# IvoteSligte/raytracing_engine

Measured on AMD Instinct MI355X. Metric: Mrays/s, higher is better.
Workload: dtype f32; 1 GPU; tri1m_1080p_4spp: 1000000 random triangles (edge +-0.08) + 1 emissive quad, single-level compressed BVH8 (249155 nodes, depth 9, one-triangle leaves), 1920x1080, 4 spp, 1 bounce + NEE, path B wavefront path tracer (camera rays: packet kernel); width=1920, height=1080, spp=4, bounces=1, tile=64, persistent_workgroups_per_cu=context default (7 for a whole frame), parallelism=single GPU, frames_in_flight=3

## Files before the change

raytracing_engine_amd/csrc/bvh_build.cpp:

```cpp
#include "bvh_build.h"

#include <algorithm>
#include <atomic>
#include <cmath>
#include <cstring>
#include <exception>
#include <limits>
#include <system_error>
#include <thread>

#include "bvh_node.h"
#include "host_parallel.h"

#ifdef RT_BVH_TIMING
#include <chrono>
#include <cstdio>
#define RT_BVH_T(x) const auto x = std::chrono::steady_clock::now()
#define RT_BVH_REPORT(what, a, b) std::fprintf(stderr, "bvh: %-18s %8.1f ms\n", what, std::chrono::duration<double, std::milli>((b) - (a)).count())
#else
#define RT_BVH_T(x) (void)0
#define RT_BVH_REPORT(what, a, b) (void)0
#endif

namespace rt {
namespace {

constexpr int kBins = 16;

struct Builder {
    const std::vector<Box>& tri_boxes;
    const std::vector<float>& centroid;
    std::vector<uint32_t>& order;
    std::vector<float>& nodes;
    float pad;
    uint32_t max_depth;
    uint32_t kLeafMax = 4;
    std::atomic<int>* spare_threads = nullptr;
    int n_threads = 1;

    struct Sub {
        int32_t ref;
        uint32_t depth_reached;
        double sah;
    };

    Box range_box(uint32_t first, uint32_t count) const {
        Box b = Box::empty();
        for (uint32_t i = 0; i < count; i++) b.grow(tri_boxes[order[first + i]]);
        return b;
    }

    void write_node(uint32_t me, const Box& b0, int32_t r0, const Box& b1, int32_t r1) {
        float* n = &nodes[(size_t)me * 16];
        const Box* side[2] = {&b0, &b1};
        for (int s = 0; s < 2; s++)
            for (int a = 0; a < 3; a++) {
                n[6 * s + a] = side[s]->lo[a] - pad;
                n[6 * s + 3 + a] = side[s]->hi[a] + pad;
            }
        std::memcpy(&n[12], &r0, 4);
        std::memcpy(&n[13], &r1, 4);
        n[14] = n[15] = 0.0f;
    }

    static int32_t leaf_ref(uint32_t first, uint32_t count) { return ~(int32_t)((first << 2) | (count - 1u)); }

    uint32_t min_depth(uint32_t count) const {
        uint32_t d = 0;
        uint64_t cap = kLeafMax;
        while (cap < count) {
            cap <<= 1;
            d++;
        }
        return d;
    }

    Sub build(uint32_t first, uint32_t count, uint32_t depth, uint32_t me) {
        if (count <= kLeafMax) return Sub{leaf_ref(first, count), 0u, 0.0};

        const int par = count >= kParallelBinMin ? n_threads : 1;
        const size_t n_chunks = (size_t)std::max(par, 1);
        const uint32_t chunk = (uint32_t)((count + n_chunks - 1) / n_chunks);
        float clo[3], chi[3];
        {
            float one_lo[3], one_hi[3];
            std::vector<float> many_lo, many_hi;
            if (n_chunks > 1) {
                many_lo.resize(3 * n_chunks);
                many_hi.resize(3 * n_chunks);
            }
            float* plo = n_chunks > 1 ? many_lo.data() : one_lo;
            float* phi = n_chunks > 1 ? many_hi.data() : one_hi;
            for (size_t i = 0; i < 3 * n_chunks; i++) {
                plo[i] = std::numeric_limits<float>::infinity();
                phi[i] = -std::numeric_limits<float>::infinity();
            }
            parallel_for(n_chunks, par, 1, [&](size_t c) {
                float lo[3] = {plo[3 * c], plo[3 * c + 1], plo[3 * c + 2]}, hi[3] = {phi[3 * c], phi[3 * c + 1], phi[3 * c + 2]};
                const uint32_t i1 = std::min<uint32_t>(count, (uint32_t)(c + 1) * chunk);
                for (uint32_t i = (uint32_t)c * chunk; i < i1; i++) {
                    const float* ce = &centroid[3 * (size_t)order[first + i]];
                    for (int a = 0; a < 3; a++) {
                        lo[a] = std::min(lo[a], ce[a]);
                        hi[a] = std::max(hi[a], ce[a]);
                    }
                }
                for (int a = 0; a < 3; a++) {
                    plo[3 * c + a] = lo[a];
                    phi[3 * c + a] = hi[a];
                }
            });
            for (int a = 0; a < 3; a++) {
                clo[a] = plo[a];
                chi[a] = phi[a];
                for (size_t c = 1; c < n_chunks; c++) {
                    clo[a] = std::min(clo[a], plo[3 * c + a]);
                    chi[a] = std::max(chi[a], phi[3 * c + a]);
                }
            }
        }

        uint32_t mid = 0;
        const bool must_balance = depth + 1 + min_depth((count + 1) / 2) >= max_depth;
        if (!must_balance) {
            float best_cost = std::numeric_limits<float>::infinity();
            int best_axis = -1, best_bin = -1;
            struct Bins {
                Box bb[3][kBins];
                uint32_t bc[3][kBins];
            };
            Bins one_part;
            std::vector<Bins> many_part;
            if (n_chunks > 1) many_part.resize(n_chunks);
            Bins* part = n_chunks > 1 ? many_part.data() : &one_part;
            float kk[3];
            for (int a = 0; a < 3; a++) kk[a] = chi[a] - clo[a] > 0.0f ? (float)kBins / (chi[a] - clo[a]) : 0.0f;
            parallel_for(n_chunks, par, 1, [&](size_t c) {
                Bins& P = part[c];
                for (int a = 0; a < 3; a++)
                    for (int b = 0; b < kBins; b++) {
                        P.bb[a][b] = Box::empty();
                        P.bc[a][b] = 0;
                    }
                const uint32_t i1 = std::min<uint32_t>(count, (uint32_t)(c + 1) * chunk);
                for (uint32_t i = (uint32_t)c * chunk; i < i1; i++) {
                    const uint32_t t = order[first + i];
                    for (int a = 0; a < 3; a++) {
                        if (!(kk[a] > 0.0f)) continue;
                        int bin = (int)((centroid[3 * (size_t)t + a] - clo[a]) * kk[a]);
                        bin = std::min(std::max(bin, 0), kBins - 1);
                        P.bb[a][bin].grow(tri_boxes[t]);
                        P.bc[a][bin]++;
                    }
                }
            });
            for (int a = 0; a < 3; a++) {
                if (!(kk[a] > 0.0f)) continue;
                Box bb[kBins];
                uint32_t bc[kBins];
                for (int b = 0; b < kBins; b++) {
                    bb[b] = part[0].bb[a][b];
                    bc[b] = part[0].bc[a][b];
                    for (size_t c = 1; c < n_chunks; c++) {
                        bb[b].grow(part[c].bb[a][b]);
                        bc[b] += part[c].bc[a][b];
                    }
                }
                float right_area[kBins];
                uint32_t right_cnt[kBins];
                Box acc = Box::empty();
                uint32_t cnt = 0;
                for (int b = kBins - 1; b > 0; b--) {
                    acc.grow(bb[b]);
                    cnt += bc[b];
                    right_area[b] = cnt ? acc.half_area() : 0.0f;
                    right_cnt[b] = cnt;
                }
                acc = Box::empty();
                cnt = 0;
                for (int b = 0; b < kBins - 1; b++) {
                    acc.grow(bb[b]);
                    cnt += bc[b];
                    if (cnt == 0 || right_cnt[b + 1] == 0) continue;
                    const float cost = acc.half_area() * (float)cnt + right_area[b + 1] * (float)right_cnt[b + 1];
                    if (cost < best_cost) {
                        best_cost = cost;
                        best_axis = a;
                        best_bin = b;
                    }
                }
            }
            if (best_axis >= 0) {
                const float k = (float)kBins / (chi[best_axis] - clo[best_axis]);
                const float lo = clo[best_axis];
                auto it = std::partition(order.begin() + first, order.begin() + first + count, [&](uint32_t t) {
                    int bin = (int)((centroid[3 * (size_t)t + best_axis] - lo) * k);
                    bin = std::min(std::max(bin, 0), kBins - 1);
                    return bin <= best_bin;
                });
                mid = (uint32_t)(it - (order.begin() + first));
                if (depth + 1 + min_depth(std::max(mid, count - mid)) >= max_depth) mid = 0;
            }
        }
        if (mid == 0 || mid == count) {
            int axis = 0;
            if (chi[1] - clo[1] > chi[axis] - clo[axis]) axis = 1;
            if (chi[2] - clo[2] > chi[axis] - clo[axis]) axis = 2;
            mid = count / 2;
            std::nth_element(order.begin() + first, order.begin() + first + mid, order.begin() + first + count,
                             [&](uint32_t x, uint32_t y) {
                                 const float cx = centroid[3 * (size_t)x + axis], cy = centroid[3 * (size_t)y + axis];
                                 return cx < cy || (cx == cy && x < y);
                             });
        }

        Box b0 = range_box(first, mid), b1 = range_box(first + mid, count - mid);
        Sub s0, s1;
        bool forked = false;
        if (spare_threads && count >= kForkMin) {
            if (spare_threads->fetch_sub(1) > 0) {
                std::exception_ptr left_err;
                std::thread left;
                try {
                    left = std::thread([&]() noexcept {
                        try {
                            s0 = build(first, mid, depth + 1, me + 1u);
                        } catch (...) {
                            left_err = std::current_exception();
                        }
                    });
                    forked = true;
                } catch (const std::system_error&) {
                }
                if (forked) {
                    {
                        struct Join {
                            std::thread& t;
                            ~Join() {
                                if (t.joinable()) t.join();
                            }
                        } join{left};
                        try {
                            s1 = build(first + mid, count - mid, depth + 1, me + mid);
                        } catch (...) {
                            spare_threads->fetch_add(1);
                            throw;
                        }
                    }
                    spare_threads->fetch_add(1);
                    if (left_err) std::rethrow_exception(left_err);
                } else {
                    spare_threads->fetch_add(1);
                }
            } else {
                spare_threads->fetch_add(1);
            }
        }
        if (!forked) {
            s0 = build(first, mid, depth + 1, me + 1u);
            s1 = build(first + mid, count - mid, depth + 1, me + mid);
        }
        write_node(me, b0, s0.ref, b1, s1.ref);
        return Sub{(int32_t)me, std::max(depth, std::max(s0.depth_reached, s1.depth_reached)),
                   ((double)b0.half_area() + (double)b1.half_area()) + (s0.sah + s1.sah)};
    }
    static constexpr uint32_t kForkMin = 1u << 14;
    static constexpr uint32_t kParallelBinMin = 1u << 17;
};

}

namespace {

struct Child {
    Box box;
    int32_t ref;
};

struct Cw8Builder {
    const std::vector<float>& n2;
    const std::vector<uint32_t>& order2;
    std::vector<uint32_t>& nodes;
    std::vector<uint32_t>& order8;
    uint32_t depth = 0;

    static constexpr float kCostNode = 1.0f;
    float kCostPrim = 0.8f;
    struct Dp {
        float cost[8];
        uint8_t split[9];
        uint8_t prev;
        uint8_t is_leaf;
        uint32_t first, prims;
        Box box;
    };
    std::vector<Dp> dp;
    int max_threads = 0;
    int thread_count() const { return max_threads > 0 ? std::min(max_threads, host_threads()) : host_threads(); }

    Box child_box(int32_t node2, int side) const {
        Box b;
        std::memcpy(b.lo, &n2[(size_t)node2 * 16 + 6 * side], 12);
        std::memcpy(b.hi, &n2[(size_t)node2 * 16 + 6 * side + 3], 12);
        return b;
    }
    int32_t child_ref(int32_t node2, int side) const {
        int32_t r;
        std::memcpy(&r, &n2[(size_t)node2 * 16 + 12 + side], 4);
        return r;
    }

    void solve() {
        const size_t n_nodes = n2.size() / 16;
        dp.resize(n_nodes);
        const int threads = thread_count();
        struct Range {
            size_t lo, hi;
        };
        std::vector<Range> subtrees;
        std::vector<size_t> top;
        const size_t grain = std::max<size_t>(n_nodes / (size_t)(8 * threads), 4096);
        std::vector<Range> todo{Range{0, n_nodes}};
        while (!todo.empty()) {
            const Range r = todo.back();
            todo.pop_back();
            if (r.hi - r.lo <= grain || threads == 1) {
                subtrees.push_back(r);
                continue;
            }
            top.push_back(r.lo);
            const int32_t r0 = child_ref((int32_t)r.lo, 0), r1 = child_ref((int32_t)r.lo, 1);
            if (r0 >= 0 && r1 >= 0) {
                todo.push_back(Range{(size_t)r0, (size_t)r1});
                todo.push_back(Range{(size_t)r1, r.hi});
            } else if (r0 >= 0) {
                todo.push_back(Range{(size_t)r0, r.hi});
            } else if (r1 >= 0) {
                todo.push_back(Range{(size_t)r1, r.hi});
            }
        }
        parallel_for(subtrees.size(), threads, 1, [&](size_t i) {
            for (size_t jj = subtrees[i].hi; jj-- > subtrees[i].lo;) solve_node(jj);
        });
        std::sort(top.begin(), top.end());
        for (size_t i = top.size(); i-- > 0;) solve_node(top[i]);
    }

    void solve_node(size_t jj) {
        {
            const int32_t j = (int32_t)jj;
            Dp& d = dp[jj];
            Box cb[2];
            float carea[2];
            int32_t cr[2];
            uint32_t cprims[2], cfirst[2];
            for (int s = 0; s < 2; s++) {
                cb[s] = child_box(j, s);
                cr[s] = child_ref(j, s);
                carea[s] = cb[s].half_area();
                if (cr[s] < 0) {
                    const uint32_t ref = ~(uint32_t)cr[s];
                    cfirst[s] = ref >> 2;
                    cprims[s] = (ref & 3u) + 1u;
                } else {
                    cfirst[s] = dp[cr[s]].first;
                    cprims[s] = dp[cr[s]].prims;
                }
            }
            auto C = [&](int s, int i) -> float {
                if (cr[s] < 0) return carea[s] * (float)cprims[s] * kCostPrim;
                return dp[cr[s]].cost[i > 7 ? 7 : i];
            };
            d.box = cb[0];
            d.box.grow(cb[1]);
            const bool same = cr[0] < 0 && cr[0] == cr[1];
            d.first = std::min(cfirst[0], cfirst[1]);
            d.prims = same ? cprims[0] : cprims[0] + cprims[1];
            float D[9];
            D[1] = std::numeric_limits<float>::infinity();
            for (int i = 2; i <= 8; i++) {
                float best = std::numeric_limits<float>::infinity();
                int bk = 1;
                for (int k = 1; k < i; k++) {
                    const float c = C(0, k) + C(1, i - k);
                    if (c < best) {
                        best = c;
                        bk = k;
                    }
                }
                D[i] = best;
                d.split[i] = (uint8_t)bk;
            }
            const float area = d.box.half_area();
            const float c_leaf = d.prims <= 1 ? area * (float)d.prims * kCostPrim : std::numeric_limits<float>::infinity();
            const float c_int = D[8] + area * kCostNode;
            d.is_leaf = c_leaf <= c_int;
            d.cost[1] = d.is_leaf ? c_leaf : c_int;
            d.prev = 0;
            for (int i = 2; i <= 7; i++) {
                if (d.cost[i - 1] <= D[i]) {
                    d.cost[i] = d.cost[i - 1];
                    d.prev |= (uint8_t)(1u << i);
                } else {
                    d.cost[i] = D[i];
                }
            }
            d.cost[0] = 0.0f;
        }
    }

    void expand(int32_t ref, const Box& box, int budget, Child* out, int& k) const {
        if (ref < 0) {
            out[k].box = box;
            out[k++].ref = ref;
            return;
        }
        const Dp& d = dp[ref];
        if (budget > 7) budget = 7;
        while (budget > 1 && ((d.prev >> budget) & 1)) budget--;
        if (budget == 1) {
            out[k].box = d.box;
            out[k++].ref = d.is_leaf ? ~(int32_t)((d.first << 2) | (d.prims - 1u)) : ref;
            return;
        }
        distribute(ref, budget, out, k);
    }
    void distribute(int32_t node2, int budget, Child* out, int& k) const {
        const int kl = dp[node2].split[budget];
        const Box b0 = child_box(node2, 0), b1 = child_box(node2, 1);
        const int32_t r0 = child_ref(node2, 0), r1 = child_ref(node2, 1);
        if (r0 < 0 && r0 == r1) {
            expand(r0, b0, 1, out, k);
            return;
        }
        expand(r0, b0, kl, out, k);
        expand(r1, b1, budget - kl, out, k);
    }

    struct Pending {
        int32_t node2;
        uint32_t index, level;
    };
    struct Work {
        Pending pd;
        Child ch[8];
        int k;
        int child_in[8];
        Box box;
        uint32_t n_inner, n_tris;
        uint32_t child_base, tri_base;
    };

    void plan(const Pending& pd, Work& w) const {
        w.pd = pd;
        Child* ch = w.ch;
        int k = 0;
        if (dp[pd.node2].is_leaf && pd.level == 0) {
            const Dp& d = dp[pd.node2];
            ch[0].box = d.box;
            ch[0].ref = ~(int32_t)((d.first << 2) | (d.prims - 1u));
            k = 1;
        } else {
            distribute(pd.node2, 8, ch, k);
        }
        w.k = k;
        Box cb[8];
        w.box = Box::empty();
        for (int i = 0; i < k; i++) {
            cb[i] = ch[i].box;
            w.box.grow(cb[i]);
        }
        assign_slots(cb, k, w.box, w.child_in);
        w.n_inner = w.n_tris = 0;
        for (int s = 0; s < 8; s++) {
            const int i = w.child_in[s];
            if (i < 0) continue;
            if (ch[i].ref >= 0) w.n_inner++;
            else w.n_tris += (~(uint32_t)ch[i].ref & 3u) + 1u;
        }
    }

    void write(const Work& wk, Pending* next_level, uint32_t next_level_base) {
        const Child* ch = wk.ch;
        Box cb[8];
        uint32_t imask = 0, leafmask = 0, rank = 0, off = 0;
        for (int s = 0; s < 8; s++) {
            const int i = wk.child_in[s];
            if (i < 0) continue;
            cb[s] = ch[i].box;
            if (ch[i].ref >= 0) {
                imask |= 1u << s;
                next_level[wk.child_base + rank - next_level_base] = Pending{ch[i].ref, wk.child_base + rank, wk.pd.level + 1};
                rank++;
            } else {
                const uint32_t ref = ~(uint32_t)ch[i].ref, first = ref >> 2;
                leafmask |= 1u << s;
                order8[(size_t)wk.tri_base + off] = order2[first];
                off += 1;
            }
        }
        uint32_t* w = node_at(nodes.data(), wk.pd.index);
        quantise(wk.box, cb, imask | leafmask, w);
        node_set_topology(w, imask, wk.child_base, wk.tri_base, leafmask);
    }

    void build() {
        RT_BVH_T(t0);
        solve();
        RT_BVH_T(t1);
        RT_BVH_REPORT("  collapse: DP", t0, t1);
        const int threads = thread_count();
        nodes.clear();
        order8.clear();
        std::vector<Pending> level{Pending{0, 0, 0}}, next;
        std::vector<Work> work;
        uint32_t node_count = 1, tri_count = 0;
        depth = 0;
        while (!level.empty()) {
            depth = level[0].level + 1;
            work.resize(level.size());
            parallel_for(level.size(), threads, 256, [&](size_t i) { plan(level[i], work[i]); });
            const uint32_t next_base = node_count;
            for (Work& w : work) {
                w.child_base = node_count;
                w.tri_base = tri_count;
                node_count += w.n_inner;
                tri_count += w.n_tris;
            }
            nodes.resize((size_t)node_count * kNodeWords, 0u);
            order8.resize(tri_count);
            next.resize(node_count - next_base);
            parallel_for(work.size(), threads, 256, [&](size_t i) { write(work[i], next.data(), next_base); });
            level.swap(next);
        }
    }
};

}

bool build_bvh(const float* v0, const float* e1, const float* e2, uint32_t n, uint32_t max_depth, BvhResult* out) {
    if (!v0 || !e1 || !e2 || n == 0 || n >= (1u << 29) || !out) return false;
    RT_BVH_T(t_start);
    std::vector<Box> tri_boxes(n);
    std::vector<float> centroid(3 * (size_t)n);
    float maxabs = 0.0f;
    for (uint32_t i = 0; i < n; i++) {
        for (int a = 0; a < 3; a++) {
            const float p0 = v0[3 * (size_t)i + a], p1 = p0 + e1[3 * (size_t)i + a], p2 = p0 + e2[3 * (size_t)i + a];
            centroid[3 * (size_t)i + a] = p0 + (e1[3 * (size_t)i + a] + e2[3 * (size_t)i + a]) * (1.0f / 3.0f);
            maxabs = std::max(maxabs, std::max(std::fabs(p0), std::max(std::fabs(p1), std::fabs(p2))));
        }
        tri_boxes[i] = tri_box(&v0[3 * (size_t)i], &e1[3 * (size_t)i], &e2[3 * (size_t)i], 0.0f);
    }
    out->order.resize(n);
    for (uint32_t i = 0; i < n; i++) out->order[i] = i;
    std::vector<float> binary;
    out->maxabs = std::max(maxabs, 1.0f);
    out->pad = out->pad_in >= 0.0f ? out->pad_in : 2e-5f * out->maxabs;
    const uint32_t leaf_max = 1;
    const int threads = out->max_threads > 0 ? std::min(out->max_threads, host_threads()) : host_threads();
    std::atomic<int> spare_threads{threads - 1};
    Builder b{tri_boxes, centroid, out->order, binary, out->pad, max_depth, leaf_max, &spare_threads, threads};
    out->sah_area = 0.0;
    if (n <= leaf_max) {
        binary.resize(16);
        const Box bx = b.range_box(0, n);
        const int32_t r = Builder::leaf_ref(0, n);
        b.write_node(0, bx, r, bx, r);
        out->depth = 1;
    } else {
        RT_BVH_T(t_prep);
        RT_BVH_REPORT("prepare", t_start, t_prep);
        binary.resize(16 * (size_t)(n - 1));
        const Builder::Sub top = b.build(0, n, 0, 0);
        out->depth = top.depth_reached + 1;
        out->sah_area = top.sah;
        RT_BVH_T(t_bin);
        RT_BVH_REPORT("binary SAH build", t_prep, t_bin);
    }
    std::vector<uint32_t> order2;
    order2.swap(out->order);
    out->order.reserve(n);
    Cw8Builder cw{binary, order2, out->nodes, out->order, 0, out->cost_prim, {}, threads};
    RT_BVH_T(t_c0);
    cw.build();
    RT_BVH_T(t_c1);
    RT_BVH_REPORT("collapse + emit", t_c0, t_c1);
    if (out->order.size() != n) return false;
    out->n_nodes = (uint32_t)(out->nodes.size() / kNodeWords);
    out->depth = cw.depth;
    out->stack_need = cw.depth + 1;
    return true;
}

}
```

raytracing_engine_amd/csrc/path_b.hip:

```cpp
#include "pt_camera.h"

namespace rt {
using namespace rtk;

__device__ __forceinline__ void sincos_2pi(float u, float& s_out, float& c_out) {
    const float t = u * 4.0f;
    uint32_t q = (uint32_t)t;
    if (q > 3u) q = 3u;
    const float th = ((t - (float)q) - 0.5f) * 1.57079632679f;
    const float th2 = th * th;
    const float ps = __builtin_fmaf(th2, __builtin_fmaf(th2, __builtin_fmaf(th2, __builtin_fmaf(th2, 2.7557319e-6f, -1.9841270e-4f), 8.3333333e-3f), -1.6666667e-1f), 1.0f);
    const float s = th * ps;
    const float c = __builtin_fmaf(th2, __builtin_fmaf(th2, __builtin_fmaf(th2, __builtin_fmaf(th2, 2.4801587e-5f, -1.3888889e-3f), 4.1666667e-2f), -0.5f), 1.0f);
    const float R = 0.70710678f;
    const float cA = (q == 0u || q == 3u) ? R : -R;
    const float sA = (q < 2u) ? R : -R;
    c_out = __builtin_fmaf(cA, c, -(sA * s));
    s_out = __builtin_fmaf(sA, c, cA * s);
}

__device__ __forceinline__ v3 cosine_dir(v3 n, float u1, float u2) {
    const float r = __builtin_sqrtf(u1);
    float s, c;
    sincos_2pi(u2, s, c);
    const float x = r * c, y = r * s, z = __builtin_sqrtf(fmax_(0.0f, 1.0f - u1));
    const float sign = n.z >= 0.0f ? 1.0f : -1.0f;
    const float a = -1.0f / (sign + n.z);
    const float b = (n.x * n.y) * a;
    const v3 b1 = mk(__builtin_fmaf(sign, (n.x * n.x) * a, 1.0f), sign * b, -sign * n.x);
    const v3 b2 = mk(b, __builtin_fmaf(n.y * n.y, a, sign), -n.y);
    return mk(__builtin_fmaf(n.x, z, __builtin_fmaf(b2.x, y, b1.x * x)), __builtin_fmaf(n.y, z, __builtin_fmaf(b2.y, y, b1.y * x)),
              __builtin_fmaf(n.z, z, __builtin_fmaf(b2.z, y, b1.z * x)));
}

__device__ __forceinline__ v3 delta_dir(v3 d, v3 n, float w, bool flipped, float u, bool& below) {
    const float c = -dot(n, d);
    below = false;
    if (w > 0.0f) {
        const float eta = flipped ? w : 1.0f / w;
        const float s2 = (eta * eta) * __builtin_fmaf(-c, c, 1.0f);
        if (s2 < 1.0f) {
            const float ct = __builtin_sqrtf(1.0f - s2);
            const float a = eta * c, b = eta * ct;
            const float rs = (a - ct) / (a + ct), rp = (c - b) / (c + b);
            const float F = __builtin_fmaf(rs, rs, rp * rp) * 0.5f;
            if (!(u < F)) {
                below = true;
                const float k = a - ct;
                return mk(__builtin_fmaf(n.x, k, eta * d.x), __builtin_fmaf(n.y, k, eta * d.y), __builtin_fmaf(n.z, k, eta * d.z));
            }
        }
    }
    return fma3(n, c + c, d);
}

constexpr uint32_t kAppendThreads = 1024;
__device__ __forceinline__ uint32_t block_append(bool want, uint32_t* counter, uint32_t* lds ) {
    const uint32_t lane = threadIdx.x & 63u, wave = threadIdx.x >> 6, n_waves = blockDim.x >> 6;
    const unsigned long long mask = __ballot(want);
    if (lane == 0) lds[wave] = (uint32_t)__popcll(mask);
    __syncthreads();
    if (threadIdx.x == 0) {
        uint32_t total = 0;
        for (uint32_t w = 0; w < n_waves; w++) total += lds[w];
        uint32_t base = total ? atomicAdd(counter, total) : 0u;
        for (uint32_t w = 0; w < n_waves; w++) {
            const uint32_t c = lds[w];
            lds[w] = base;
            base += c;
        }
    }
    __syncthreads();
    const uint32_t idx = lds[wave] + (uint32_t)__popcll(mask & ((1ull << lane) - 1ull));
    __syncthreads();
    return idx;
}

constexpr uint32_t kSortBins = 512;
template <uint32_t BINS = kSortBins>
__device__ __forceinline__ uint32_t block_append_sorted(bool want, uint32_t key, uint32_t* counter, uint32_t* lds) {
    static_assert(BINS % 64u == 0u && BINS <= kSortBins, "whole waves of bins");
    uint32_t* hist = lds;
    uint32_t* wsum = lds + kSortBins;
    for (uint32_t i = threadIdx.x; i < BINS; i += blockDim.x) hist[i] = 0;
    __syncthreads();
    uint32_t rank = 0;
    if (want) rank = atomicAdd(&hist[key], 1u);
    __syncthreads();
    const uint32_t lane = threadIdx.x & 63u, wave = threadIdx.x >> 6;
    uint32_t v = 0, incl = 0;
    if (threadIdx.x < BINS) {
        v = hist[threadIdx.x];
        incl = v;
        for (int off = 1; off < 64; off <<= 1) {
            const uint32_t t = __shfl_up(incl, off);
            if ((int)lane >= off) incl += t;
        }
        if (lane == 63) wsum[wave] = incl;
    }
    __syncthreads();
    if (threadIdx.x == 0) {
        uint32_t total = 0;
        for (uint32_t w = 0; w < BINS / 64u; w++) {
            const uint32_t c = wsum[w];
            wsum[w] = total;
            total += c;
        }
        wsum[16] = total ? atomicAdd(counter, total) : 0u;
    }
    __syncthreads();
    if (threadIdx.x < BINS) hist[threadIdx.x] = wsum[wave] + incl - v;
    __syncthreads();
    const uint32_t idx = want ? wsum[16] + hist[key] + rank : 0u;
    __syncthreads();
    return idx;
}

__device__ __forceinline__ uint32_t ray_sort_key(const float4* __restrict__ nodes, v3 o, v3 d) {
    const float4 n0 = nodes[0];
    const uint32_t w3 = __float_as_uint(n0.w);
    const float ex = __uint_as_float((((w3 & 0xffu) + 6u) & 0xffu) << 23), ey = __uint_as_float(((((w3 >> 8) & 0xffu) + 6u) & 0xffu) << 23),
                ez = __uint_as_float(((((w3 >> 16) & 0xffu) + 6u) & 0xffu) << 23);
    const int cx = (int)((o.x - n0.x) / ex), cy = (int)((o.y - n0.y) / ey), cz = (int)((o.z - n0.z) / ez);
    const uint32_t ux = (uint32_t)(cx < 0 ? 0 : cx > 3 ? 3 : cx), uy = (uint32_t)(cy < 0 ? 0 : cy > 3 ? 3 : cy), uz = (uint32_t)(cz < 0 ? 0 : cz > 3 ? 3 : cz);
    const uint32_t oct = (__float_as_uint(d.x) >> 31) | ((__float_as_uint(d.y) >> 31) << 1) | ((__float_as_uint(d.z) >> 31) << 2);
    return (oct << 6) | (uz << 4) | (uy << 2) | ux;
}

__device__ __forceinline__ uint32_t shadow_work_key(v3 d) {
    const float l2 = dot(d, d);
    const int e = (int)((__float_as_uint(l2) >> 21) & 0x3ffu) - (125 << 2);
    return (uint32_t)(e < 0 ? 0 : e > 63 ? 63 : e);
}
__device__ __forceinline__ uint32_t bounce_work_key(v3 d) {
    const float ax = __builtin_fabsf(d.x), ay = __builtin_fabsf(d.y), az = __builtin_fabsf(d.z);
    const uint32_t axis = ax >= ay && ax >= az ? 0u : ay >= az ? 1u : 2u;
    const float m = axis == 0u ? ax : axis == 1u ? ay : az;
    const int q = (int)((m - 0.5f) * 32.0f);
    return axis * 16u + (uint32_t)(q < 0 ? 0 : q > 15 ? 15 : q);
}

__global__ __launch_bounds__(kAppendThreads) void pt_generate(const PtFrame f, PtState st, uint32_t* __restrict__ queue, uint32_t* __restrict__ ctr) {
    __shared__ uint32_t lds[32];
    const uint32_t pid = blockIdx.x * kAppendThreads + threadIdx.x;
    bool alive = false;
    if (pid < f.n_paths) {
        const uint32_t slot = pid / f.spp_batch, s = f.sample0 + (pid - slot * f.spp_batch);
        uint32_t px, py, lx, ly, k;
        if (slot_pixel(f, slot, px, py, lx, ly, k)) {
            alive = true;
            const v3 d = camera_dir(f, px, py, s);
            st.ray_o[pid] = make_float4(f.cam.pos[0], f.cam.pos[1], f.cam.pos[2], 0.0f);
            st.ray_d[pid] = make_float4(d.x, d.y, d.z, 0.0f);
            st.thr[pid] = make_float4(1.0f, 1.0f, 1.0f, 0.0f);
        }
        st.rad[pid] = make_float4(0.0f, 0.0f, 0.0f, 0.0f);
    }
    const uint32_t idx = block_append(alive, &ctr[PT_CTR_COUNT], lds);
    if (alive) queue[idx] = pid;
}

template <bool SURF>
__global__ __launch_bounds__(kAppendThreads, 8) void pt_shade(const PtScene sc, const PtFrame f, PtState st, const uint32_t* __restrict__ queue,
                                                           const uint32_t* __restrict__ count_ptr, uint32_t depth, uint32_t* __restrict__ next_queue,
                                                           uint32_t* __restrict__ next_ctr, uint32_t sort_rays) {
    __shared__ uint32_t lds[kSortBins + 40];
    const bool direct = queue == nullptr;
    const uint32_t n = direct ? f.n_paths : *count_ptr;
    const uint32_t stride = gridDim.x * kAppendThreads;
    for (uint32_t base = blockIdx.x * kAppendThreads; base < n; base += stride) {
        const uint32_t i = base + threadIdx.x;
        bool bounce = false, shadow = false;
        uint32_t pid = 0;
        float4 so = {}, sd = {}, scn = {};
        bool item = i < n;
        if (item && direct) {
            uint32_t px, py, lx, ly, k;
            item = slot_pixel(f, i / f.spp_batch, px, py, lx, ly, k);
        }
        if (item) {
            pid = direct ? i : queue[i];
            const float2 hrec = st.hit[pid];
            const int li = __float_as_int(hrec.y);
            const float4 rd = st.ray_d[pid];
            const float4 ro = direct ? make_float4(f.cam.pos[0], f.cam.pos[1], f.cam.pos[2], 0.0f) : st.ray_o[pid];
            const float4 T = direct ? make_float4(1.0f, 1.0f, 1.0f, 0.0f) : st.thr[pid];
            const v3 o = mk(ro.x, ro.y, ro.z), d = mk(rd.x, rd.y, rd.z);
            float4 L = direct ? make_float4(0.0f, 0.0f, 0.0f, 0.0f) : st.rad[pid];
            if (direct) st.rad[pid] = L;
            if (li < 0) {
                L.x = __builtin_fmaf(T.x, f.sky[0], L.x);
                L.y = __builtin_fmaf(T.y, f.sky[1], L.y);
                L.z = __builtin_fmaf(T.z, f.sky[2], L.z);
                st.rad[pid] = L;
            } else {
                const float4 ta = sc.tris[(size_t)li * 3 + 0], tb = sc.tris[(size_t)li * 3 + 1], tc = sc.tris[(size_t)li * 3 + 2];
                if (__float_as_uint(tc.z) != 0u) {
                    if (depth == 0 || (SURF && T.w != 0.0f)) {
                        const float4 em = sc.emission[li];
                        L.x = __builtin_fmaf(T.x, em.x, L.x);
                        L.y = __builtin_fmaf(T.y, em.y, L.y);
                        L.z = __builtin_fmaf(T.z, em.z, L.z);
                        st.rad[pid] = L;
                    }
                } else {
                    const float4 alb = sc.albedo[li];
                    v3 nrm = normalize(cross(mk(ta.w, tb.x, tb.y), mk(tb.z, tb.w, tc.x)));
                    const bool flipped = dot(nrm, d) > 0.0f;
                    if (flipped) nrm = -nrm;
                    const v3 pt = fma3(d, hrec.x, o);
                    const v3 po = fma3(nrm, f.ray_eps, pt);
                    const uint32_t slot = pid / f.spp_batch, s = f.sample0 + (pid - slot * f.spp_batch);
                    uint32_t px, py, lx, ly, k;
                    slot_pixel(f, slot, px, py, lx, ly, k);
                    const uint32_t key = path_key(py * f.width + px, s, f.seed);
                    const bool delta = SURF && alb.w != 0.0f;
                    if (delta && depth < f.bounces) {
                        bool below;
                        const v3 nd = delta_dir(d, nrm, alb.w, flipped, rnd(key, depth, 7), below);
                        const v3 no = below ? fma3(nrm, -f.ray_eps, pt) : po;
                        bounce = true;
                        st.ray_o[pid] = make_float4(no.x, no.y, no.z, 0.0f);
                        st.ray_d[pid] = make_float4(nd.x, nd.y, nd.z, 0.0f);
                        st.thr[pid] = make_float4(T.x * alb.x, T.y * alb.y, T.z * alb.z, 1.0f);
                    }
                    if (!delta && sc.n_lights > 0) {
                        uint32_t kk = (uint32_t)(rnd(key, depth, 2) * (float)sc.n_lights);
                        if (kk > sc.n_lights - 1) kk = sc.n_lights - 1;
                        const uint32_t lt = sc.lights[kk];
                        const float su = __builtin_sqrtf(rnd(key, depth, 3)), u2 = rnd(key, depth, 4);
                        const float b1 = su * (1.0f - u2), b2 = su * u2;
                        const float4 la = sc.tris[(size_t)lt * 3 + 0], lb = sc.tris[(size_t)lt * 3 + 1], lc = sc.tris[(size_t)lt * 3 + 2];
                        const v3 lv0 = mk(la.x, la.y, la.z), le1 = mk(la.w, lb.x, lb.y), le2 = mk(lb.z, lb.w, lc.x);
                        const v3 q = mk(__builtin_fmaf(le2.x, b2, __builtin_fmaf(le1.x, b1, lv0.x)), __builtin_fmaf(le2.y, b2, __builtin_fmaf(le1.y, b1, lv0.y)),
                                        __builtin_fmaf(le2.z, b2, __builtin_fmaf(le1.z, b1, lv0.z)));
                        const v3 wi = q - po;
                        const float d2 = dot(wi, wi);
                        const v3 nl = cross(le1, le2);
                        const float cs = dot(nrm, wi), cl = __builtin_fabsf(dot(nl, wi));
                        const float d4 = d2 * d2;
                        if (cs > 0.0f && cl > 0.0f && d4 > 0.0f) {
                            const float w = ((cs * cl) * ((float)sc.n_lights * 0.15915494f)) / d4;
                            const float4 le = sc.emission[lt];
                            shadow = true;
                            so = make_float4(po.x, po.y, po.z, __uint_as_float(pid));
                            sd = make_float4(wi.x, wi.y, wi.z, 0.0f);
                            scn = make_float4(((T.x * alb.x) * le.x) * w, ((T.y * alb.y) * le.y) * w, ((T.z * alb.z) * le.z) * w, 0.0f);
                        }
                    }
                    if (!delta && depth < f.bounces) {
                        const v3 nd = cosine_dir(nrm, rnd(key, depth, 5), rnd(key, depth, 6));
                        bounce = true;
                        st.ray_o[pid] = make_float4(po.x, po.y, po.z, 0.0f);
                        st.ray_d[pid] = make_float4(nd.x, nd.y, nd.z, 0.0f);
                        st.thr[pid] = make_float4(T.x * alb.x, T.y * alb.y, T.z * alb.z, 0.0f);
                    }
                }
            }
        }
        uint32_t bi, si;
        if (sort_rays == 2u) {
            uint32_t kb = 0, ks = 0;
            if (bounce) {
                const float4 rd = st.ray_d[pid];
                kb = bounce_work_key(mk(rd.x, rd.y, rd.z));
            }
            if (shadow) ks = shadow_work_key(mk(sd.x, sd.y, sd.z));
            bi = block_append_sorted<64>(bounce, kb, &next_ctr[PT_CTR_COUNT], lds);
            si = block_append_sorted<64>(shadow, ks, &next_ctr[PT_CTR_SHADOW_COUNT], lds);
        } else if (sort_rays) {
            uint32_t kb = 0, ks = 0;
            if (bounce) {
                const float4 ro = st.ray_o[pid], rd = st.ray_d[pid];
                kb = ray_sort_key(sc.nodes, mk(ro.x, ro.y, ro.z), mk(rd.x, rd.y, rd.z));
            }
            if (shadow) ks = ray_sort_key(sc.nodes, mk(so.x, so.y, so.z), mk(sd.x, sd.y, sd.z));
            bi = block_append_sorted(bounce, kb, &next_ctr[PT_CTR_COUNT], lds);
            si = block_append_sorted(shadow, ks, &next_ctr[PT_CTR_SHADOW_COUNT], lds);
        } else {
            bi = block_append(bounce, &next_ctr[PT_CTR_COUNT], lds);
            si = block_append(shadow, &next_ctr[PT_CTR_SHADOW_COUNT], lds);
        }
        if (bounce) next_queue[bi] = pid;
        if (shadow) {
            st.sh_o[si] = so;
            st.sh_d[si] = sd;
            st.sh_c[si] = scn;
        }
    }
}

__global__ __launch_bounds__(256) void pt_resolve(const PtFrame f, PtState st, float* __restrict__ acc, float* __restrict__ dst, uint32_t tile_major) {
    const uint32_t slot = blockIdx.x * 256u + threadIdx.x;
    if (slot >= f.n_slots) return;
    uint32_t px, py, lx, ly, k;
    if (!slot_pixel(f, slot, px, py, lx, ly, k)) return;
    float r = 0.0f, g = 0.0f, b = 0.0f;
    if (f.sample0 > 0) {
        r = acc[(size_t)slot * 3 + 0];
        g = acc[(size_t)slot * 3 + 1];
        b = acc[(size_t)slot * 3 + 2];
    }
    for (uint32_t s = 0; s < f.spp_batch; s++) {
        const float4 L = st.rad[(size_t)slot * f.spp_batch + s];
        r += L.x;
        g += L.y;
        b += L.z;
    }
    if (f.sample0 + f.spp_batch < f.spp_total) {
        acc[(size_t)slot * 3 + 0] = r;
        acc[(size_t)slot * 3 + 1] = g;
        acc[(size_t)slot * 3 + 2] = b;
        return;
    }
    const float inv = (float)f.spp_total;
    const size_t idx = tile_major ? ((size_t)k * (RT_TILE * RT_TILE) + (size_t)ly * RT_TILE + lx) : ((size_t)py * f.width + px);
    dst[idx * 3 + 0] = r / inv;
    dst[idx * 3 + 1] = g / inv;
    dst[idx * 3 + 2] = b / inv;
}

__global__ __launch_bounds__(256) void pt_scatter_surfaces(const float4* __restrict__ tris, const float* __restrict__ surf, float4* __restrict__ albedo,
                                                           uint32_t n) {
    const uint32_t li = blockIdx.x * 256u + threadIdx.x;
    if (li >= n) return;
    const uint32_t t = __float_as_uint(tris[(size_t)li * 3 + 2].y);
    reinterpret_cast<float*>(albedo)[(size_t)li * 4 + 3] = surf && t < n ? surf[t] : 0.0f;
}

int launch_pt_generate(Ctx* c, const PtFrame& f, const PtState& st, uint32_t* queue, uint32_t* ctr) {
    hipLaunchKernelGGL(pt_generate, dim3((f.n_paths + kAppendThreads - 1u) / kAppendThreads), dim3(kAppendThreads), 0, c->stream, f, st, queue, ctr);
    RT_HIP(c, hipGetLastError());
    return RT_OK;
}

int launch_pt_shade(Ctx* c, const PtScene& sc, const PtFrame& f, const PtState& st, const uint32_t* queue, const uint32_t* count_ptr,
                    uint32_t depth, uint32_t* next_queue, uint32_t* next_ctr, uint32_t grid, uint32_t sort_rays, bool surfaces) {
    if (surfaces)
        hipLaunchKernelGGL(pt_shade<true>, dim3(grid), dim3(kAppendThreads), 0, c->stream, sc, f, st, queue, count_ptr, depth, next_queue, next_ctr,
                           sort_rays);
    else
        hipLaunchKernelGGL(pt_shade<false>, dim3(grid), dim3(kAppendThreads), 0, c->stream, sc, f, st, queue, count_ptr, depth, next_queue, next_ctr,
                           sort_rays);
    RT_HIP(c, hipGetLastError());
    return RT_OK;
}

int launch_pt_scatter_surfaces(Ctx* c, const float4* tris, const float* surf, float4* albedo, uint32_t n) {
    hipLaunchKernelGGL(pt_scatter_surfaces, dim3((n + 255u) / 256u), dim3(256), 0, c->stream, tris, surf, albedo, n);
    RT_HIP(c, hipGetLastError());
    return RT_OK;
}

int launch_pt_resolve(Ctx* c, const PtFrame& f, const PtState& st, float* acc, float* dst, int tile_major) {
    hipLaunchKernelGGL(pt_resolve, dim3((f.n_slots + 255u) / 256u), dim3(256), 0, c->stream, f, st, acc, dst, (uint32_t)(tile_major ? 1 : 0));
    RT_HIP(c, hipGetLastError());
    return RT_OK;
}

}
```

Baseline: 2905 Mrays/s.

## Cache light triangles in LDS, hoist hit loads, and double BVH SAH bins

When the scene has at most 32 lights, the shade kernel now loads their triangle and emission data into shared memory once per workgroup and reads from there during light sampling. Hit-triangle and albedo loads are issued early and pinned with empty asm barriers so their latency overlaps other work. For scenes with many lights, light selection is computed up front. Separately, the BVH builder uses 32 SAH bins instead of 16, which changes tree quality and traversal cost, and the sort-append helper pins threadIdx in a register.

Result: faster. 2957 Mrays/s (median of 6 runs) (+1.8%).

```diff
diff --git a/raytracing_engine_amd/csrc/bvh_build.cpp b/raytracing_engine_amd/csrc/bvh_build.cpp
--- a/raytracing_engine_amd/csrc/bvh_build.cpp
+++ b/raytracing_engine_amd/csrc/bvh_build.cpp
@@ -25,7 +25,7 @@
 namespace rt {
 namespace {
 
-constexpr int kBins = 16;
+constexpr int kBins = 32;
 
 struct Builder {
     const std::vector<Box>& tri_boxes;
diff --git a/raytracing_engine_amd/csrc/path_b.hip b/raytracing_engine_amd/csrc/path_b.hip
--- a/raytracing_engine_amd/csrc/path_b.hip
+++ b/raytracing_engine_amd/csrc/path_b.hip
@@ -82,15 +82,17 @@
     static_assert(BINS % 64u == 0u && BINS <= kSortBins, "whole waves of bins");
     uint32_t* hist = lds;
     uint32_t* wsum = lds + kSortBins;
-    for (uint32_t i = threadIdx.x; i < BINS; i += blockDim.x) hist[i] = 0;
+    uint32_t tid = threadIdx.x;
+    asm volatile("" : "+v"(tid));
+    for (uint32_t i = tid; i < BINS; i += blockDim.x) hist[i] = 0;
     __syncthreads();
     uint32_t rank = 0;
     if (want) rank = atomicAdd(&hist[key], 1u);
     __syncthreads();
-    const uint32_t lane = threadIdx.x & 63u, wave = threadIdx.x >> 6;
+    const uint32_t lane = tid & 63u, wave = tid >> 6;
     uint32_t v = 0, incl = 0;
-    if (threadIdx.x < BINS) {
-        v = hist[threadIdx.x];
+    if (tid < BINS) {
+        v = hist[tid];
         incl = v;
         for (int off = 1; off < 64; off <<= 1) {
             const uint32_t t = __shfl_up(incl, off);
@@ -99,7 +101,7 @@
         if (lane == 63) wsum[wave] = incl;
     }
     __syncthreads();
-    if (threadIdx.x == 0) {
+    if (tid == 0) {
         uint32_t total = 0;
         for (uint32_t w = 0; w < BINS / 64u; w++) {
             const uint32_t c = wsum[w];
@@ -109,7 +111,7 @@
         wsum[16] = total ? atomicAdd(counter, total) : 0u;
     }
     __syncthreads();
-    if (threadIdx.x < BINS) hist[threadIdx.x] = wsum[wave] + incl - v;
+    if (tid < BINS) hist[tid] = wsum[wave] + incl - v;
     __syncthreads();
     const uint32_t idx = want ? wsum[16] + hist[key] + rank : 0u;
     __syncthreads();
@@ -160,58 +162,81 @@
     if (alive) queue[idx] = pid;
 }
 
-template <bool SURF>
+constexpr uint32_t kShadeLightTable = 32;
+__device__ __forceinline__ void keep_here(float& x) { asm volatile("" : "+v"(x)); }
+__device__ __forceinline__ uint32_t light_pick(const PtScene& sc, const PtFrame& f, uint32_t pid, uint32_t depth) {
+    const uint32_t slot = pid / f.spp_batch, s = f.sample0 + (pid - slot * f.spp_batch);
+    uint32_t px, py, lx, ly, k;
+    slot_pixel(f, slot, px, py, lx, ly, k);
+    const uint32_t kk = (uint32_t)(rnd(path_key(py * f.width + px, s, f.seed), depth, 2) * (float)sc.n_lights);
+    return kk > sc.n_lights - 1 ? sc.n_lights - 1 : kk;
+}
+template <bool SURF, bool TAB>
 __global__ __launch_bounds__(kAppendThreads, 8) void pt_shade(const PtScene sc, const PtFrame f, PtState st, const uint32_t* __restrict__ queue,
                                                            const uint32_t* __restrict__ count_ptr, uint32_t depth, uint32_t* __restrict__ next_queue,
                                                            uint32_t* __restrict__ next_ctr, uint32_t sort_rays) {
     __shared__ uint32_t lds[kSortBins + 40];
+    __shared__ float4 light_tab[kShadeLightTable * 4];
     const bool direct = queue == nullptr;
     const uint32_t n = direct ? f.n_paths : *count_ptr;
     const uint32_t stride = gridDim.x * kAppendThreads;
+    if (TAB) {
+        if (threadIdx.x < sc.n_lights * 4u) {
+            const uint32_t lt = sc.lights[threadIdx.x >> 2], j = threadIdx.x & 3u;
+            float4 v = j < 3u ? sc.tris[(size_t)lt * 3 + j] : sc.emission[lt];
+            if (j == 3u) v.w = __uint_as_float(lt);
+            light_tab[threadIdx.x] = v;
+        }
+        __syncthreads();
+    }
     for (uint32_t base = blockIdx.x * kAppendThreads; base < n; base += stride) {
         const uint32_t i = base + threadIdx.x;
         bool bounce = false, shadow = false;
         uint32_t pid = 0;
         float4 so = {}, sd = {}, scn = {};
         bool item = i < n;
-        if (item && direct) {
-            uint32_t px, py, lx, ly, k;
-            item = slot_pixel(f, i / f.spp_batch, px, py, lx, ly, k);
-        }
+        uint32_t px = 0, py = 0, lx, ly, k;
+        if (item && direct) item = slot_pixel(f, i / f.spp_batch, px, py, lx, ly, k);
         if (item) {
             pid = direct ? i : queue[i];
             const float2 hrec = st.hit[pid];
-            const int li = __float_as_int(hrec.y);
+            uint32_t lt = 0;
+            if (!TAB) lt = sc.lights[light_pick(sc, f, pid, depth)];
             const float4 rd = st.ray_d[pid];
             const float4 ro = direct ? make_float4(f.cam.pos[0], f.cam.pos[1], f.cam.pos[2], 0.0f) : st.ray_o[pid];
             const float4 T = direct ? make_float4(1.0f, 1.0f, 1.0f, 0.0f) : st.thr[pid];
+            float4 L = direct ? make_float4(0.0f, 0.0f, 0.0f, 0.0f) : st.rad[pid];
+            const int li = __float_as_int(hrec.y);
+            const size_t lr = li < 0 ? 0 : (size_t)li;
+            float4 ta = sc.tris[lr * 3 + 0], tb = sc.tris[lr * 3 + 1], tc = sc.tris[lr * 3 + 2];
+            float4 alb = sc.albedo[lr];
+            keep_here(tc.z), keep_here(ta.w), keep_here(tb.x), keep_here(tb.y), keep_here(tb.z), keep_here(tb.w), keep_here(tc.x);
+            keep_here(alb.x), keep_here(alb.y), keep_here(alb.z);
+            if (SURF) keep_here(alb.w);
             const v3 o = mk(ro.x, ro.y, ro.z), d = mk(rd.x, rd.y, rd.z);
-            float4 L = direct ? make_float4(0.0f, 0.0f, 0.0f, 0.0f) : st.rad[pid];
-            if (direct) st.rad[pid] = L;
             if (li < 0) {
                 L.x = __builtin_fmaf(T.x, f.sky[0], L.x);
                 L.y = __builtin_fmaf(T.y, f.sky[1], L.y);
                 L.z = __builtin_fmaf(T.z, f.sky[2], L.z);
                 st.rad[pid] = L;
             } else {
-                const float4 ta = sc.tris[(size_t)li * 3 + 0], tb = sc.tris[(size_t)li * 3 + 1], tc = sc.tris[(size_t)li * 3 + 2];
                 if (__float_as_uint(tc.z) != 0u) {
-                    if (depth == 0 || (SURF && T.w != 0.0f)) {
+                    const bool seen = depth == 0 || (SURF && T.w != 0.0f);
+                    if (seen) {
                         const float4 em = sc.emission[li];
                         L.x = __builtin_fmaf(T.x, em.x, L.x);
                         L.y = __builtin_fmaf(T.y, em.y, L.y);
                         L.z = __builtin_fmaf(T.z, em.z, L.z);
-                        st.rad[pid] = L;
                     }
+                    if (seen || direct) st.rad[pid] = L;
                 } else {
-                    const float4 alb = sc.albedo[li];
+                    if (direct) st.rad[pid] = L;
                     v3 nrm = normalize(cross(mk(ta.w, tb.x, tb.y), mk(tb.z, tb.w, tc.x)));
                     const bool flipped = dot(nrm, d) > 0.0f;
                     if (flipped) nrm = -nrm;
                     const v3 pt = fma3(d, hrec.x, o);
                     const v3 po = fma3(nrm, f.ray_eps, pt);
                     const uint32_t slot = pid / f.spp_batch, s = f.sample0 + (pid - slot * f.spp_batch);
-                    uint32_t px, py, lx, ly, k;
                     slot_pixel(f, slot, px, py, lx, ly, k);
                     const uint32_t key = path_key(py * f.width + px, s, f.seed);
                     const bool delta = SURF && alb.w != 0.0f;
@@ -225,12 +250,19 @@
                         st.thr[pid] = make_float4(T.x * alb.x, T.y * alb.y, T.z * alb.z, 1.0f);
                     }
                     if (!delta && sc.n_lights > 0) {
-                        uint32_t kk = (uint32_t)(rnd(key, depth, 2) * (float)sc.n_lights);
-                        if (kk > sc.n_lights - 1) kk = sc.n_lights - 1;
-                        const uint32_t lt = sc.lights[kk];
+                        float4 la, lb, lc, le;
+                        if (TAB) {
+                            uint32_t kk = (uint32_t)(rnd(key, depth, 2) * (float)sc.n_lights);
+                            if (kk > sc.n_lights - 1) kk = sc.n_lights - 1;
+                            la = light_tab[kk * 4u + 0u], lb = light_tab[kk * 4u + 1u], lc = light_tab[kk * 4u + 2u];
+                            le = light_tab[kk * 4u + 3u];
+                        } else {
+                            la = sc.tris[(size_t)lt * 3 + 0], lb = sc.tris[(size_t)lt * 3 + 1], lc = sc.tris[(size_t)lt * 3 + 2];
+                            le = sc.emission[lt];
+                            keep_here(le.x), keep_here(le.y), keep_here(le.z);
+                        }
                         const float su = __builtin_sqrtf(rnd(key, depth, 3)), u2 = rnd(key, depth, 4);
                         const float b1 = su * (1.0f - u2), b2 = su * u2;
-                        const float4 la = sc.tris[(size_t)lt * 3 + 0], lb = sc.tris[(size_t)lt * 3 + 1], lc = sc.tris[(size_t)lt * 3 + 2];
                         const v3 lv0 = mk(la.x, la.y, la.z), le1 = mk(la.w, lb.x, lb.y), le2 = mk(lb.z, lb.w, lc.x);
                         const v3 q = mk(__builtin_fmaf(le2.x, b2, __builtin_fmaf(le1.x, b1, lv0.x)), __builtin_fmaf(le2.y, b2, __builtin_fmaf(le1.y, b1, lv0.y)),
                                         __builtin_fmaf(le2.z, b2, __builtin_fmaf(le1.z, b1, lv0.z)));
@@ -241,7 +273,6 @@
                         const float d4 = d2 * d2;
                         if (cs > 0.0f && cl > 0.0f && d4 > 0.0f) {
                             const float w = ((cs * cl) * ((float)sc.n_lights * 0.15915494f)) / d4;
-                            const float4 le = sc.emission[lt];
                             shadow = true;
                             so = make_float4(po.x, po.y, po.z, __uint_as_float(pid));
                             sd = make_float4(wi.x, wi.y, wi.z, 0.0f);
@@ -336,12 +367,9 @@
 
 int launch_pt_shade(Ctx* c, const PtScene& sc, const PtFrame& f, const PtState& st, const uint32_t* queue, const uint32_t* count_ptr,
                     uint32_t depth, uint32_t* next_queue, uint32_t* next_ctr, uint32_t grid, uint32_t sort_rays, bool surfaces) {
-    if (surfaces)
-        hipLaunchKernelGGL(pt_shade<true>, dim3(grid), dim3(kAppendThreads), 0, c->stream, sc, f, st, queue, count_ptr, depth, next_queue, next_ctr,
-                           sort_rays);
-    else
-        hipLaunchKernelGGL(pt_shade<false>, dim3(grid), dim3(kAppendThreads), 0, c->stream, sc, f, st, queue, count_ptr, depth, next_queue, next_ctr,
-                           sort_rays);
+    const bool tab = sc.n_lights <= kShadeLightTable;
+    auto kernel = surfaces ? (tab ? pt_shade<true, true> : pt_shade<true, false>) : (tab ? pt_shade<false, true> : pt_shade<false, false>);
+    hipLaunchKernelGGL(kernel, dim3(grid), dim3(kAppendThreads), 0, c->stream, sc, f, st, queue, count_ptr, depth, next_queue, next_ctr, sort_rays);
     RT_HIP(c, hipGetLastError());
     return RT_OK;
 }
```
